# ssydasheng/GPflow-Slim

Measured on AMD Instinct MI355X. Metric: GPR log-marginal-likelihood evals/sec + predict_f latency, fp64, N=32768 D=8, higher is better.
Workload: dtype f64; 1 GPU; RBF(ARD) GPR log-marginal-likelihood, N=32768 D=8 R=1 fp64, X resident in HBM; n=32768, d=8, n_new=1024, parallelism=1 GPU (fused single-GPU path)

## Files before the change

gpflow-slim_amd/csrc/blas1.hip:

```cpp
#include "gps_common.hpp"

typedef double v2d __attribute__((ext_vector_type(2)));

__device__ __forceinline__ double wave_sum(double v) {
#pragma unroll
  for (int off = 32; off > 0; off >>= 1) v += __shfl_xor(v, off, 64);
  return v;
}

__global__ __launch_bounds__(256) void trsv_base_kernel(const double* __restrict__ LinvT,
                                                        double* __restrict__ y, i64 ldy) {
  __shared__ double ys[128];
  __shared__ double part[128];
  double* yr = y + (i64)blockIdx.x * ldy;
  const int tid = threadIdx.x, i = tid & 127, half = tid >> 7;
  if (tid < 128) ys[tid] = yr[tid];
  __syncthreads();
  const double* Lc = LinvT + (half * 64) * 128 + i;
  double s = 0.0;
#pragma unroll 16
  for (int c = 0; c < 64; ++c) s += Lc[c * 128] * ys[half * 64 + c];
  if (half) part[i] = s;
  __syncthreads();
  if (!half) yr[i] = s + part[i];
}

template <int RC>
__global__ __launch_bounds__(256) void gemv_sub_kernel(const double* __restrict__ L21, i64 ldl,
                                                       i64 n2, i64 n1,
                                                       const double* __restrict__ y1,
                                                       double* __restrict__ y2, i64 ldy, int r0,
                                                       int rcount) {
  const int lane = threadIdx.x & 63;
// ... 549 lines not shown
  const i64 row = (i64)blockIdx.x * 4 + (threadIdx.x >> 6);
  if (row >= rows) return;
  const double* a = A + row * lda; const double* b = B + row * ldb;
  double s = 0.0;
  for (i64 k = 2 * lane; k < cols; k += 128) {
    const v2d x = *reinterpret_cast<const v2d*>(a + k), y = *reinterpret_cast<const v2d*>(b + k);
    s = fma(x.x, y.x, fma(x.y, y.y, s));
  }
  s = wave_sum(s);
  if (lane == 0) out[row] = s;
}
__global__ __launch_bounds__(256) void rows_axpby_kernel(double* __restrict__ X, i64 ldx, const double* __restrict__ Y, i64 ldy,
                                                         i64 rows, i64 cols, const double* __restrict__ a, const double* __restrict__ b) {
  const i64 c = (i64)blockIdx.x * blockDim.x + threadIdx.x;
  if (c >= cols) return;
  for (i64 rr = blockIdx.y; rr < rows; rr += gridDim.y) X[rr * ldx + c] = a[rr] * X[rr * ldx + c] + b[rr] * Y[rr * ldy + c];
}
int gps_launch_rowdot2(gps_handle_t h, const double* A, i64 lda, const double* B, i64 ldb, i64 rows, i64 cols, double* out) {
  if (rows <= 0 || cols <= 0) return GPS_OK;
  LaunchScope ls(h, KC_REDUCE, 2.0 * rows * cols, 16.0 * rows * cols);
  hipLaunchKernelGGL(rowdot2_kernel, dim3((unsigned)((rows + 3) / 4)), dim3(256), 0, h->stream, A, lda, B, ldb, rows, cols, out);
  GPS_HIP(h, hipGetLastError());
  return GPS_OK;
}
int gps_launch_rows_axpby(gps_handle_t h, double* X, i64 ldx, const double* Y, i64 ldy, i64 rows, i64 cols, const double* a,
                          const double* b) {
  if (rows <= 0 || cols <= 0) return GPS_OK;
  LaunchScope ls(h, KC_OTHER, 3.0 * rows * cols, 24.0 * rows * cols);
  dim3 grid((unsigned)((cols + 255) / 256), (unsigned)(rows < 32768 ? rows : 32768));
  hipLaunchKernelGGL(rows_axpby_kernel, grid, dim3(256), 0, h->stream, X, ldx, Y, ldy, rows, cols, a, b);
  GPS_HIP(h, hipGetLastError());
  return GPS_OK;
}
int gps_launch_axpby_eye(gps_handle_t h, double* A, i64 ld, i64 n, i64 n_real, double alpha, double beta) {
  if (n <= 0) return GPS_OK;
  LaunchScope ls(h, KC_OTHER, (double)n * n, 16.0 * n * n);
  dim3 grid((unsigned)((n + 255) / 256), (unsigned)(n < 32768 ? n : 32768));
  hipLaunchKernelGGL(axpby_eye_kernel, grid, dim3(256), 0, h->stream, A, ld, n, n_real, alpha, beta);
  GPS_HIP(h, hipGetLastError());
  return GPS_OK;
}
int gps_launch_diag_recip_add(gps_handle_t h, double* A, i64 lda, const double* L, i64 ldl, i64 n, double coef) {
  if (n <= 0) return GPS_OK;
  hipLaunchKernelGGL(diag_recip_add_kernel, dim3((unsigned)((n + 255) / 256)), dim3(256), 0, h->stream, A, lda, L, ldl, n, coef);
  GPS_HIP(h, hipGetLastError());
  return GPS_OK;
}
int gps_tri_dot(gps_handle_t h, const double* A, i64 lda, const double* B, i64 ldb, i64 n, double* out2) {
  out2[0] = out2[1] = 0.0;
  if (n <= 0) return GPS_OK;
  double* part = h->dScal.d();
  {
    LaunchScope ls(h, KC_REDUCE, (double)n * n, 8.0 * n * n);
    hipLaunchKernelGGL(tri_dot_kernel, dim3(64), dim3(256), 0, h->stream, A, lda, B, ldb, n, part);
    GPS_HIP(h, hipGetLastError());
  }
  double hp[128];
  GPS_HIP(h, hipMemcpyAsync(hp, part, sizeof(hp), hipMemcpyDeviceToHost, h->stream));
  GPS_HIP(h, hipStreamSynchronize(h->stream));
  for (int b = 0; b < 64; ++b) { out2[0] += hp[2 * b]; out2[1] += hp[2 * b + 1]; }
  return GPS_OK;
}

int gps_launch_tri_map(gps_handle_t h, double* A, i64 ld, i64 n, int mode) {
  if (n <= 0) return GPS_OK;
  LaunchScope ls(h, KC_OTHER, (double)n * n, 16.0 * n * n);
// ... 169 lines not shown
```

gpflow-slim_amd/csrc/gemm_f64.hip:

```cpp
#include "gps_common.hpp"

typedef double v4d __attribute__((ext_vector_type(4)));
typedef double v2d __attribute__((ext_vector_type(2)));

#define BK_MIN 16
#ifndef STRIP
#define STRIP 8
#endif

struct GemmArgs {
  const double* A; const double* B; double* C;
  i64 lda, ldb, ldc;
  int Tm, Tn;
  int K;
  int ntiles;
  int triA;
  int batch, tpb;
  int pair;
  i64 a_rs, a_cs, b_rs, b_cs, c_rs, c_cs, a_cm, b_cm, c_cm;
  int cb_tiles;
  i64 cb_stride;
  int cb_cpack = 0;
  int nfull, nsplit;
  double* ws;
  unsigned* cnt;
  unsigned long long* sig_ptr; unsigned long long sig_val;
  long long* stamps;
};

__device__ __forceinline__ int xcd_remap(int b, int nb) {
#ifdef GPS_GEMM_NO_XCD_REMAP
  return b;
#endif
  const int q = nb >> 3, r = nb & 7;
  const int x = b & 7, idx = b >> 3;
  const int base = (x < r) ? x * (q + 1) : r * (q + 1) + (x - r) * q;
  return base + idx;
}

template <bool LOWER>
__device__ __forceinline__ void decode_tile(int id, int Tm, int Tn, int& tm, int& tn) {
  if (!LOWER) {
    const int full = Tn / STRIP;
    const int per = Tm * STRIP;
    int s = id / per;
    if (s >= full) {
      const int w = Tn - full * STRIP;
      const int rem = id - full * per;
      tm = rem / w; tn = full * STRIP + rem % w;
    } else {
      const int rem = id - s * per;
      tm = rem / STRIP; tn = s * STRIP + rem % STRIP;
    }
  } else {
    int s = 0, rem = id;
    for (;;) {
      const int c0 = s * STRIP;
      const int w = min(STRIP, Tn - c0);
      const int tri = w * (w + 1) / 2;
      const int cnt = tri + (Tm - c0 - w) * w;
      if (rem < cnt) {
        if (rem < tri) {
          int rr = 0;
          while (rem >= rr + 1) { rem -= rr + 1; ++rr; }
          tm = c0 + rr; tn = c0 + rem;
        } else {
          rem -= tri;
          tm = c0 + w + rem / w; tn = c0 + rem % w;
        }
        return;
      }
      rem -= cnt; ++s;
    }
  }
}

#define GEMM_KERNEL_NAME gemm_nt_f64_kernel
#define GEMM_PAIR_TPARAM
#include "gemm_f64_kernel.inc"
#undef GEMM_KERNEL_NAME
#undef GEMM_PAIR_TPARAM
#define GEMM_PAIRED
#define GEMM_KERNEL_NAME gemm_nt_f64_pair_kernel
#define GEMM_PAIR_TPARAM , int PAIR = 1
#include "gemm_f64_kernel.inc"
#undef GEMM_PAIRED
#undef GEMM_KERNEL_NAME
#undef GEMM_PAIR_TPARAM

template <int BM, int BN, int WGM, bool LOWER, int OP, int PIPE = 0, int BKT = 16>
static int launch_variant(gps_handle_t h, const GemmArgs& g) {
  const size_t lds = (size_t)(2 * (BM + BN) * (BKT + 2)) * sizeof(double);
  if (g.pair && BM == BN && PIPE == 2 && !LOWER && (OP == 1 || OP == 3)) {
    const int grid = g.ntiles;
    if (g.pair == 1) {
      int rc = gps_dyn_lds(h, reinterpret_cast<const void*>(&gemm_nt_f64_pair_kernel<BM, BN, WGM, false, OP, PIPE, BKT, 1>), (int)lds);
      if (rc) return rc;
      hipLaunchKernelGGL((gemm_nt_f64_pair_kernel<BM, BN, WGM, false, OP, PIPE, BKT, 1>), dim3(grid), dim3(256), lds, h->stream, g);
    } else {
      int rc = gps_dyn_lds(h, reinterpret_cast<const void*>(&gemm_nt_f64_pair_kernel<BM, BN, WGM, false, OP, PIPE, BKT, 2>), (int)lds);
      if (rc) return rc;
      hipLaunchKernelGGL((gemm_nt_f64_pair_kernel<BM, BN, WGM, false, OP, PIPE, BKT, 2>), dim3(grid), dim3(256), lds, h->stream, g);
    }
    GPS_HIP(h, hipGetLastError());
    return GPS_OK;
  }
  int rc = gps_dyn_lds(h, reinterpret_cast<const void*>(&gemm_nt_f64_kernel<BM, BN, WGM, LOWER, OP, PIPE, BKT>), (int)lds);
  if (rc) return rc;
  const int grid = g.nsplit > 1 ? g.nfull + (g.ntiles - g.nfull) * g.nsplit : g.ntiles;
  hipLaunchKernelGGL((gemm_nt_f64_kernel<BM, BN, WGM, LOWER, OP, PIPE, BKT>), dim3(grid), dim3(256), lds, h->stream, g);
  GPS_HIP(h, hipGetLastError());
// ... 98 lines not shown
  g.cb_tiles = 0; g.cb_stride = 0;
  const double t128 = (double)nbatch * (lower ? 0.5 * (double)(N / 128) * (double)(N / 128 + 1) + (double)((M - N) / 128) * (double)(N / 128)
                                             : ((double)M / 128.0) * (double)(N / 128));
  const double flops = triA == 3 ? (double)nbatch * 128.0 * 128.0 * ((double)M / 128.0) * (double)(N / 128) * (double)(N + 128)
                     : triA      ? (double)nbatch * 128.0 * 128.0 * (double)(N / 128) * (double)(M / 128) * (double)(M + 128)
                                 : 2.0 * t128 * 128.0 * 128.0 * (double)K;
  const double bytes = t128 * (((op == 0 || op == 2) ? 2.0 : 1.0) * 128.0 * 128.0 * 8.0) +
                       8.0 * (double)K * (double)(M + N);
  LaunchScope ls(h, KC_GEMM, flops, bytes);
  ls.tag[0] = M; ls.tag[1] = N; ls.tag[2] = K; ls.tag[3] = op + 10 * lower + 20 * triA + 100 * (rowpanel ? 1 : 0) + 1000 * (nbatch > 1 ? nbatch : 0);
  const double target = (double)h->gemm_min_tiles;
  const int force = h->gemm_force_tb;
  if (rowpanel) {
    int bm = 16;
    if (force) bm = (half_rows && force > 64) ? 64 : force;
    else if (M / 128 >= 256 && !half_rows) bm = 128;
    else if (M / 64 >= 256) bm = 64;
    else if (M / 32 >= 256) bm = 32;
    if (bm == 128) return launch_cfg<128, 128, 2>(h, op, 0, g, M, N);
    if (bm == 64) return launch_cfg<64, 128, 2>(h, op, 0, g, M, N);
    if (bm == 32) return launch_cfg<32, 128, 1>(h, op, 0, g, M, N);
    return launch_cfg<16, 128, 1>(h, op, 0, g, M, N);
  }
  int tb = 32;
  if (force) tb = force < 32 ? 32 : force;
  else if (t128 >= target && !half_rows) tb = 128;
  else if (4.0 * t128 >= target) tb = 64;
  if (half_rows && tb > 64) tb = 64;
  if (tb == 128) return launch_cfg<128, 128, 2>(h, op, lower, g, M, N);
  if (tb == 64) return launch_cfg<64, 64, 2>(h, op, lower, g, M, N);
  return launch_cfg<32, 32, 2>(h, op, lower, g, M, N);
}

int gps_launch_gemm_nt_cyclic(gps_handle_t h, i64 M, i64 nblocks, i64 nb, i64 stride, i64 K, const double* A, i64 lda,
                              double* C, i64 ldc, int c_packed) {
  if (M <= 0 || nblocks <= 0) return GPS_OK;
  if (M % 128 || nb % 128 || stride % 128 || K % BK_MIN || stride < nb || (nblocks - 1) * stride + nb > M)
    return gps_fail(h, GPS_ERR_ARG, "gemm_nt_cyclic: sizes must be multiples of 128 and the blocks must lie inside the panel");
  GemmArgs g;
  g.A = A; g.B = A; g.C = C; g.lda = lda; g.ldb = lda; g.ldc = ldc; g.K = (int)K; g.triA = 0;
  g.batch = 1; g.tpb = 0; g.pair = 0; g.a_rs = g.a_cs = g.b_rs = g.b_cs = g.c_rs = g.c_cs = g.a_cm = g.b_cm = g.c_cm = 0;
  g.sig_ptr = nullptr; g.sig_val = 0;
  g.stamps = h->gemm_stamps;
  double t128 = 0.0;
  for (i64 b = 0; b < nblocks; ++b) { const i64 rows = M - b * stride; if (rows > 0) t128 += (double)(rows / 128) * (double)(nb / 128); }
  const double flops = 2.0 * t128 * 128.0 * 128.0 * (double)K;
  LaunchScope ls(h, KC_GEMM, flops, t128 * 2.0 * 128.0 * 128.0 * 8.0 + 8.0 * (double)K * (double)(M + nblocks * nb));
  const double target = (double)h->gemm_min_tiles;
  g.cb_stride = stride;
  g.cb_cpack = c_packed ? 1 : 0;
  if (t128 >= target) { g.cb_tiles = (int)(nb / 128); return launch_cfg<128, 128, 2>(h, 0, 0, g, M, nblocks * nb); }
  if (4.0 * t128 >= target) { g.cb_tiles = (int)(nb / 64); return launch_cfg<64, 64, 2>(h, 0, 0, g, M, nblocks * nb); }
  g.cb_tiles = (int)(nb / 32);
  return launch_cfg<32, 32, 2>(h, 0, 0, g, M, nblocks * nb);
}
```

gpflow-slim_amd/csrc/gemm_f64_kernel.inc:

```
template <int BM, int BN, int WGM, bool LOWER, int OP, int PIPE = 0, int BKT = 16 GEMM_PAIR_TPARAM>
__global__ __launch_bounds__(256, 2) void GEMM_KERNEL_NAME(GemmArgs g) {
  constexpr int BK = BKT, LS = BKT + 2;
  constexpr int TPR = BKT / 2, RPP = 256 / TPR;
  constexpr int WGN = 4 / WGM;
  constexpr int WTM = BM / WGM, WTN = BN / WGN;
  constexpr int MI = WTM / 16, NI = WTN / 16;
  constexpr int LPA = (BM + RPP - 1) / RPP, LPB = (BN + RPP - 1) / RPP;
  static_assert(MI >= 1 && NI >= 1, "wave tile must hold at least one MFMA tile");
  constexpr int KS = (MI * NI >= 4) ? 1 : (MI * NI == 2 ? 2 : 4);
  extern __shared__ __attribute__((aligned(16))) char smem_raw[];
  double* As = reinterpret_cast<double*>(smem_raw);
  double* Bs = As + 2 * BM * LS;

  int tile_id, slice = -1, tail = 0;
  if ((int)blockIdx.x < g.nfull || g.nsplit <= 1) {
    tile_id = xcd_remap((int)blockIdx.x, g.nsplit > 1 ? g.nfull : g.ntiles);
  } else {
    const int q = (int)blockIdx.x - g.nfull;
    tail = q / g.nsplit;
    slice = q - tail * g.nsplit;
    tile_id = g.nfull + tail;
  }
  int tm, tn;
  i64 bcol;
  const double* gA = g.A; const double* gB = g.B; double* gC = g.C;
  if (g.batch > 1) {
    const int p = tile_id / g.tpb;
    tile_id -= p * g.tpb;
    gA += (i64)p * g.a_rs * g.lda + (g.a_cm ? ((i64)p * g.a_cs) % g.a_cm : (i64)p * g.a_cs);
    gB += (i64)p * g.b_rs * g.ldb + (g.b_cm ? ((i64)p * g.b_cs) % g.b_cm : (i64)p * g.b_cs);
    gC += (i64)p * g.c_rs * g.ldc + (g.c_cm ? ((i64)p * g.c_cs) % g.c_cm : (i64)p * g.c_cs);
  }
  if (g.cb_tiles > 0) {
    const int q = (int)(g.cb_stride / BM);
// ... 228 lines not shown
          for (int rg = 0; rg < 4; ++rg) acc[0][i][j][rg] += v[i][j][rg];
    }
    if (tid == 0) g.cnt[tail] = 0;
  }
  const i64 row0 = (i64)tm * BM + wr * WTM + (lane >> 4);
  const i64 col0 = (g.cb_cpack ? (i64)tn * BN : bcol) + wc * WTN + (lane & 15);
  constexpr int IB = (MI >= 2) ? 2 : 1;
#pragma unroll
  for (int i0 = 0; i0 < MI; i0 += IB) {
    double cv[IB][NI][4];
    if (OP == 0 || OP == 2) {
#pragma unroll
      for (int ii = 0; ii < IB; ++ii)
#pragma unroll
        for (int j = 0; j < NI; ++j)
#pragma unroll
          for (int rg = 0; rg < 4; ++rg)
            cv[ii][j][rg] = gC[(row0 + (i0 + ii) * 16 + 4 * rg) * g.ldc + col0 + j * 16];
    }
#pragma unroll
    for (int ii = 0; ii < IB; ++ii)
#pragma unroll
      for (int j = 0; j < NI; ++j)
#pragma unroll
        for (int rg = 0; rg < 4; ++rg) {
          double* cp = gC + (row0 + (i0 + ii) * 16 + 4 * rg) * g.ldc + col0 + j * 16;
          const double av = acc[0][i0 + ii][j][rg];
          if (OP == 0) *cp = cv[ii][j][rg] - av;
          else if (OP == 2) *cp = cv[ii][j][rg] + av;
          else if (OP == 3) *cp = -av;
          else *cp = av;
        }
  }
#ifdef GEMM_PAIRED
  }
#endif
  if (g.stamps && threadIdx.x == 0) g.stamps[6 * (long long)blockIdx.x + 1] = (long long)wall_clock64();
}
```

gpflow-slim_amd/csrc/gps_common.hpp:

```cpp
#pragma once
#include <hip/hip_runtime.h>
#include <cstdint>
#include <cstdio>
#include <cstring>
#include <cstdlib>
#include <string>
#include <vector>
#include "../../include/gpflowslim_hip.h"
#include "blocked.hpp"

#define GPS_TILE 128
#define GPS_WB 2048
#define GPS_WIDE_MAX_ROWS 8192

typedef int64_t i64;

static inline i64 gps_pad(i64 n) { return ((n + GPS_TILE - 1) / GPS_TILE) * GPS_TILE; }

struct DevBuf;
typedef std::vector<DevBuf*> DevBufList;
struct DevBuf {
  enum Class { WORK, PERSISTENT };
  void*  p = nullptr;
  size_t cap = 0;
// ... 172 lines not shown
  DevBuf dA{bufs};
  DevBuf dY{bufs};
  DevBuf dKinv{bufs};
  DevBuf dS1{bufs}, dS2{bufs}, dS3{bufs}, dS4{bufs};
  DevBuf dG1{bufs}, dG2{bufs}, dG3{bufs}, dG4{bufs};
  DevBuf dLikIn{bufs}, dLikOut{bufs}, dLikPart{bufs}, dLikH{bufs};
  DevBuf dTmp{bufs};
  DevBuf dTmp2{bufs};
  DevBuf dTmp3{bufs};
  static constexpr long long resid_ring_max = 1 << 16;
  int trsm_panel = 1;
  int trsm_tall_ratio = 16;
  int trsm_panel_rows = 0;
  DevBuf dSmallOut{bufs};
  DevBuf dFeatG{bufs};
  DevBuf dGradSums{bufs};
  void* hRes = nullptr;
  DevBuf dBlkCond{bufs};
  DevBuf dSmallSync{bufs, DevBuf::PERSISTENT};
  static constexpr i64 small_n_max = 2048;
  struct SmallPath {
    int on = 1;
    int fault_inject = 0;
    long long fallbacks = 0;
    int consec = 0;
    int cooldown = 0;
    bool defer = false;
    bool pending = false;
    bool valid = false;
    double slog = 0.0, ssq = 0.0;
    bool linvT_stale = false;
  } small;
  DevBuf dGemmWs{bufs}, dGemmCnt{bufs};
  struct RffFactor { bool have = false; unsigned long long gen = 0; i64 F = 0, r = 0; int kind = -1, d = 0; bool refine = false; } rff;
  DevBuf dGemvWs{bufs}, dGemvCnt{bufs};
  struct KgprSolve { bool have = false; unsigned long long gen = 0; i64 m = 0, n = 0; } kgpr;
  int kron_cg_check_every = 8;
};

static inline int gps_fail(gps_handle_t h, int code, const std::string& msg) {
  if (h) h->err = msg;
  return code;
}

static inline int gps_dyn_lds(gps_handle_t h, const void* fn, int bytes);

#define GPS_HIP(h, call)                                                         \
  do {                                                                           \
    hipError_t e__ = (call);                                                     \
    if (e__ != hipSuccess) {                                                     \
      return gps_fail(h, GPS_ERR_HIP, std::string(#call) + ": " + hipGetErrorString(e__)); \
    }                                                                            \
  } while (0)

static inline void drop_resident_factors(gps_handle_t h) {
  h->have_factor = false; h->factor_gen++; h->dist.have_part_factor = false; h->dist.grad_ready = false;
}

#define DIST_TAIL 4
struct DistPanel {
  i64 np, nb, ld;
  i64 rows;
  i64 blk0, nbb;
  i64 below;
  double* panel;
  i64 inv_doubles() const { return nbb * GPS_TILE * GPS_TILE; }
// ... 52 lines not shown
    hipEvent_t e; (void)hipEventCreate(&e); return e;
  }
};

static inline void gps_profile_collect(gps_handle_t h) {
  static const char* dump_path = getenv("GPS_PROF_DUMP");
  FILE* df = (dump_path && !h->pending.empty()) ? fopen(dump_path, "a") : nullptr;
  for (auto& p : h->pending) {
    float ms = 0.f;
    if (hipEventElapsedTime(&ms, p.a, p.b) == hipSuccess) h->stat[p.klass].ms += ms;
    if (df) fprintf(df, "%s %lld %lld %lld %lld %.3f\n", kc_names[p.klass], (long long)p.t[0], (long long)p.t[1], (long long)p.t[2], (long long)p.t[3], 1e3 * ms);
    h->evt_pool.push_back(p.a); h->evt_pool.push_back(p.b);
  }
  if (df) fclose(df);
  h->pending.clear();
}

static inline int gps_dyn_lds(gps_handle_t h, const void* fn, int bytes) {
  for (const void* f : h->dyn_lds_done) if (f == fn) return GPS_OK;
  GPS_HIP(h, hipFuncSetAttribute(fn, hipFuncAttributeMaxDynamicSharedMemorySize, bytes));
  h->dyn_lds_done.push_back(fn);
  return GPS_OK;
}

int gps_launch_gemm_nt(gps_handle_t h, int op, int lower, i64 M, i64 N, i64 K,
                       const double* A, i64 lda, const double* B, i64 ldb,
                       double* C, i64 ldc);
struct GemmBatch;
int gps_launch_gemm_nt_ex(gps_handle_t h, int op, int lower, int tri, i64 M, i64 N, i64 K,
                          const double* A, i64 lda, const double* B, i64 ldb,
                          double* C, i64 ldc, const GemmBatch* bt);
int gps_launch_gemm_nt_cyclic(gps_handle_t h, i64 M, i64 nblocks, i64 nb, i64 stride, i64 K, const double* A, i64 lda,
                              double* C, i64 ldc, int c_packed = 0);
int gps_launch_potrf_base(gps_handle_t h, double* A, i64 lda, double* Linv_blk,
                          double* LinvT_blk, int* d_info, i64 row0, int factor,
                          long long* d_stamps = nullptr);
int gps_launch_trsm_leaf_refine(gps_handle_t h, double* B, i64 ldb, i64 m, const double* W, const double* D, i64 ldd,
                                int upper);
int gps_launch_trsv_leaf_refine(gps_handle_t h, const double* Wt, const double* D, i64 ldd, double* y, i64 ldy, i64 r,
                                int upper);
static inline bool gps_gpr_needs_refine(const gps_handle_s* h, double noise_var, double kdiag, i64 n) {
  if (h->leaf_refine >= 0) return h->leaf_refine > 0;
  return !((double)n * kdiag + noise_var <= h->leaf_refine_cond * noise_var);
}

struct SmallKgen { int on = 0; int op = 0; const double* X = nullptr; int d_all = 0; int nd = 0; int dims[16]; double inv_ls[16]; double variance = 0.0, noise = 0.0; };
int gps_launch_small_factor(gps_handle_t h, double* dK, i64 np, double* linv, double* linvT, const double* d_resid, i64 n, i64 r,
                            int* d_info, double* d_res4, double* d_alpha, i64 ld_alpha, i64 alpha_rows, const SmallKgen* kgen = nullptr);
int gps_small_factor_reset(gps_handle_t h);
int gps_launch_trsm_panel(gps_handle_t h, double* B, i64 ldb, i64 m, const double* L, i64 ldl, const double* W, int backward);
int gps_launch_small_inverse(gps_handle_t h, const double* dK, i64 np, const double* linv, const double* d_alpha, i64 r,
                             double* dY, double* dKinv, double* dA, double* d_res1, double* dAT = nullptr, i64 n = 0);
int gps_launch_trsv_wave(gps_handle_t h, const double* L, i64 ldl, i64 n, const double* W, double* y, i64 ldy, i64 r,
                         int trans, int refine = 0);
int gps_launch_trsv_base(gps_handle_t h, const double* Linv_blk, double* y, i64 ldy, i64 r);
int gps_launch_la_wait(gps_handle_t h, hipStream_t st, unsigned long long* sig, unsigned long long sval,
                       const unsigned long long* flag, unsigned long long val, unsigned long long* timeouts);
int gps_launch_gemv_sub(gps_handle_t h, const double* L21, i64 ldl, i64 n2, i64 n1,
                        const double* y1, double* y2, i64 ldy, i64 r);
int gps_launch_gemv_t_sub(gps_handle_t h, const double* L21, i64 ldl, i64 n2, i64 n1,
                          const double* y2, double* y1, i64 ldy, i64 r);
int gps_launch_lml_reduce(gps_handle_t h, const double* L, i64 ldl, i64 n,
                          const double* alpha, i64 ldy, i64 r, double* out2);
int gps_launch_colsumsq(gps_handle_t h, const double* A, i64 ld, i64 rows, i64 cols, double* sumsq);
int gps_launch_rowdot(gps_handle_t h, const double* At, i64 ldat, i64 n_new, i64 npad,
                      const double* alpha, i64 ldy, i64 r, double* mean, double* sumsq);
// ... 118 lines not shown
```

gpflow-slim_amd/csrc/gps_handle.hip:

```cpp
#include "gps_ops.hpp"

extern "C" int gps_create(int device_id, gps_handle_t* out) {
  if (!out) return GPS_ERR_ARG;
  *out = nullptr;
  int count = 0;
  if (hipGetDeviceCount(&count) != hipSuccess || count <= 0) return GPS_ERR_HIP;
  if (device_id < 0 || device_id >= count) return GPS_ERR_ARG;
  gps_handle_t h = new gps_handle_s();
  h->device = device_id;
  if (hipSetDevice(device_id) != hipSuccess || hipGetDeviceProperties(&h->prop, device_id) != hipSuccess) {
    delete h;
    return GPS_ERR_HIP;
  }
  if (hipStreamCreateWithFlags(&h->stream, hipStreamNonBlocking) != hipSuccess) { delete h; return GPS_ERR_HIP; }
  for (int i = 0; i < 8; ++i) {
    if (hipEventCreate(&h->ev[i]) != hipSuccess) { delete h; return GPS_ERR_HIP; }
  }
  if (const char* v = getenv("GPS_GEMM_PAIR")) h->gemm_pair = atoi(v);
  if (const char* la = getenv("GPS_LOOKAHEAD")) h->potrf_lookahead = atoi(la);
  if (h->dInfo.ensure(64) != hipSuccess || h->dScal.ensure(4096) != hipSuccess) { delete h; return GPS_ERR_HIP; }
  *out = h;
  return GPS_OK;
}

// ... 77 lines not shown
    {"trsv_wave_fallbacks", (long long)h->wave_fallbacks},
  };
  for (const auto& c : counters) {
    if (strcmp(klass, c.key) != 0) continue;
    if (launches) *launches = (int64_t)c.value;
    if (ms) *ms = 0.0;
    if (flops) *flops = 0.0;
    if (bytes) *bytes = 0.0;
    return GPS_OK;
  }
  GPS_HIP(h, hipStreamSynchronize(h->stream));
  gps_profile_collect(h);
  for (int i = 0; i < KC_COUNT; ++i) {
    if (strcmp(klass, kc_names[i]) == 0) {
      if (launches) *launches = h->stat[i].launches;
      if (ms) *ms = h->stat[i].ms;
      if (flops) *flops = h->stat[i].flops;
      if (bytes) *bytes = h->stat[i].bytes;
      return GPS_OK;
    }
  }
  return gps_fail(h, GPS_ERR_ARG, "unknown kernel class");
}
extern "C" int gps_last_stage_ms(gps_handle_t h, double* out5) {
  if (!h || !out5) return GPS_ERR_ARG;
  for (int i = 0; i < 5; ++i) out5[i] = h->stage_ms[i];
  return GPS_OK;
}

extern "C" int gps_set_option(gps_handle_t h, const char* key, double value) {
  if (!h || !key) return GPS_ERR_ARG;
  if (strcmp(key, "gemm_force_tile") == 0) { h->gemm_force_tb = (int)value; return GPS_OK; }
  if (strcmp(key, "gemm_tail_split") == 0) { h->gemm_tail_split = (int)value; return GPS_OK; }
  if (strcmp(key, "kmat_fast") == 0) { h->kmat_fast = (int)value; return GPS_OK; }
  if (strcmp(key, "kmat_mfma") == 0) { h->kmat_mfma = (int)value; return GPS_OK; }
  if (strcmp(key, "trsv_wave") == 0) { h->trsv_wave = (int)value; return GPS_OK; }
  if (strcmp(key, "gpr_aug_rows") == 0) { h->gpr_aug_rows = (int)value; return GPS_OK; }
  if (strcmp(key, "leaf_refine") == 0) { h->leaf_refine = (int)value; return GPS_OK; }
  if (strcmp(key, "potrf_rl_max") == 0) { h->potrf_rl_max = (int)value; return GPS_OK; }
  if (strcmp(key, "potrf_lookahead") == 0) { h->potrf_lookahead = (int)value; return GPS_OK; }
  if (strcmp(key, "la_fault_inject") == 0) { h->la_fault_inject = (int)value; return GPS_OK; }
  if (strcmp(key, "wave_fault_inject") == 0) { h->wave_fault_inject = (int)value; return GPS_OK; }
  if (strcmp(key, "small_fault_inject") == 0) { h->small.fault_inject = (int)value; return GPS_OK; }
  if (strcmp(key, "svgp_kl_weight") == 0) { h->svgp_kl_weight = value; return GPS_OK; }
  if (strcmp(key, "dist_partitioned") == 0) { h->dist.partitioned = (int)value; return GPS_OK; }
  if (strcmp(key, "leaf_plain_kappa") == 0) { h->leaf_plain_kappa = value; h->plain_linv = nullptr; return GPS_OK; }
  if (strcmp(key, "follower_max_wgs") == 0) { h->follower_max_wgs = (int)value; return GPS_OK; }
  if (strcmp(key, "potrf_rl_group") == 0) { h->potrf_rl_group = (int)value < 1 ? 1 : (int)value; return GPS_OK; }
  if (strcmp(key, "small_n") == 0) { h->small.on = (int)value; return GPS_OK; }
  if (strcmp(key, "trsm_panel") == 0) { h->trsm_panel = (int)value; return GPS_OK; }
  if (strcmp(key, "trsm_tall_ratio") == 0) { h->trsm_tall_ratio = (int)value; return GPS_OK; }
  if (strcmp(key, "trsm_panel_rows") == 0) {
    if (value != 0 && value != 32 && value != 64 && value != 65) return gps_fail(h, GPS_ERR_ARG, "trsm_panel_rows: 0, 32, 64 or 65");
    h->trsm_panel_rows = (int)value; return GPS_OK;
  }
  if (strcmp(key, "predict_inverse_blocks") == 0) { h->predict_inv_blocks = (int)value; return GPS_OK; }
  if (strcmp(key, "trsv_wave_refine") == 0) { h->trsv_wave_refine = (int)value; return GPS_OK; }
  if (strcmp(key, "kron_cg_check_every") == 0) { h->kron_cg_check_every = (int)value < 1 ? 1 : (int)value; return GPS_OK; }
  return gps_fail(h, GPS_ERR_ARG, "unknown option");
}

extern "C" int gps_diag_mfma_f64(gps_handle_t h, int waves_per_simd, double* tflops, int* layout_ok) {
  if (!h) return GPS_ERR_ARG;
  GPS_HIP(h, hipSetDevice(h->device));
  return gps_run_mfma_diag(h, waves_per_simd, tflops, layout_ok);
}

extern "C" int gps_diag_gemm_nt(gps_handle_t h, int op, int lower, int64_t m, int64_t n, int64_t k,
                                const double* A, const double* B, double* C) {
  if (!h || !A || !B || !C) return GPS_ERR_ARG;
  GPS_HIP(h, hipSetDevice(h->device));
  const size_t ab = (size_t)m * k * 8, bb = (size_t)n * k * 8, cb = (size_t)m * n * 8;
  GPS_HIP(h, h->dTmp.ensure(ab)); GPS_HIP(h, h->dTmp2.ensure(bb)); GPS_HIP(h, h->dTmp3.ensure(cb));
  GPS_HIP(h, hipMemcpyAsync(h->dTmp.p, A, ab, hipMemcpyHostToDevice, h->stream));
  GPS_HIP(h, hipMemcpyAsync(h->dTmp2.p, B, bb, hipMemcpyHostToDevice, h->stream));
  GPS_HIP(h, hipMemcpyAsync(h->dTmp3.p, C, cb, hipMemcpyHostToDevice, h->stream));
  int rc = lower >= 3 ? gps_launch_gemm_nt_ex(h, op, 0, lower - 1, m, n, k, h->dTmp.d(), k, h->dTmp2.d(), k, h->dTmp3.d(), n, nullptr)
                      : gps_launch_gemm_nt(h, op, lower, m, n, k, h->dTmp.d(), k, h->dTmp2.d(), k, h->dTmp3.d(), n);
  if (rc) return rc;
  GPS_HIP(h, hipMemcpyAsync(C, h->dTmp3.p, cb, hipMemcpyDeviceToHost, h->stream));
  GPS_HIP(h, hipStreamSynchronize(h->stream));
  return GPS_OK;
}

extern "C" int gps_diag_gemm_nt_batched(gps_handle_t h, int op, int tri, int64_t batch, int64_t m, int64_t n, int64_t k,
                                        const double* A, const double* B, double* C) {
  if (!h || !A || !B || !C || batch < 1) return GPS_ERR_ARG;
  GPS_HIP(h, hipSetDevice(h->device));
  const size_t ab = (size_t)batch * m * k * 8, bb = (size_t)batch * n * k * 8, cb = (size_t)batch * m * n * 8;
  GPS_HIP(h, h->dTmp.ensure(ab)); GPS_HIP(h, h->dTmp2.ensure(bb)); GPS_HIP(h, h->dTmp3.ensure(cb));
  GPS_HIP(h, hipMemcpyAsync(h->dTmp.p, A, ab, hipMemcpyHostToDevice, h->stream));
  GPS_HIP(h, hipMemcpyAsync(h->dTmp2.p, B, bb, hipMemcpyHostToDevice, h->stream));
  GPS_HIP(h, hipMemcpyAsync(h->dTmp3.p, C, cb, hipMemcpyHostToDevice, h->stream));
  GemmBatch bt; bt.batch = batch; bt.a_rs = m; bt.b_rs = n; bt.c_rs = m;
  int rc = gps_launch_gemm_nt_ex(h, op, 0, tri, m, n, k, h->dTmp.d(), k, h->dTmp2.d(), k, h->dTmp3.d(), n, &bt);
  if (rc) return rc;
  GPS_HIP(h, hipMemcpyAsync(C, h->dTmp3.p, cb, hipMemcpyDeviceToHost, h->stream));
  GPS_HIP(h, hipStreamSynchronize(h->stream));
  return GPS_OK;
}

extern "C" int gps_diag_gemm_timeline(gps_handle_t h, int op, int lower, int64_t m, int64_t n, int64_t k, int reps,
                                      long long* stamps_out, int64_t cap_blocks, int64_t* nblocks, double* ms_per_launch) {
  if (!h || !stamps_out || cap_blocks <= 0 || reps <= 0) return GPS_ERR_ARG;
  GPS_HIP(h, hipSetDevice(h->device));
  return gps_run_gemm_timeline(h, op, lower, m, n, k, reps, stamps_out, cap_blocks, nblocks, ms_per_launch);
}

extern "C" int gps_diag_potrf_base_stamps(gps_handle_t h, int factor, double* us_out7) {
  if (!h || !us_out7) return GPS_ERR_ARG;
  GPS_HIP(h, hipSetDevice(h->device));
// ... 231 lines not shown
```

gpflow-slim_amd/csrc/gps_ops.hpp:

```cpp
#pragma once
#include "gps_common.hpp"
#include "blocked.hpp"
#include "dist_schedule.hpp"
#include <climits>
#include <cmath>
#include <algorithm>

struct HipOps {
  gps_handle_t h;
  double* linv;
  double* linvT;
  int* d_info;
  int factor = 1;
  bool store_T = true;

  int potrf_base(double* A, i64 lda, i64 blk, i64 row0) {
    if (h->plain_linv == linv) h->plain_linv = nullptr;
    return gps_launch_potrf_base(h, A, lda, linv + blk * GPS_TILE * GPS_TILE,
                                 (linvT && store_T) ? linvT + blk * GPS_TILE * GPS_TILE : nullptr, d_info, row0,
                                 factor);
  }
  int trsm_base(i64 blk, int transposed, double* B, i64 ldb, i64 m, const double* D, i64 ldd) {
    const double* W = (transposed ? linvT : linv) + blk * GPS_TILE * GPS_TILE;
    if (h->refine_now && !plain_ok(blk, 1)) { h->leaves_refined++; return gps_launch_trsm_leaf_refine(h, B, ldb, m, W, D, ldd, transposed); }
    if (h->refine_now) h->leaves_plain++;
    return gps_launch_gemm_nt(h,  1, 0, m, GPS_TILE, GPS_TILE, B, ldb, W, GPS_TILE, B, ldb);
  }
  bool plain_ok(i64 blk, i64 cnt) const {
    if (h->plain_linv != linv || blk < 0 || (size_t)(blk + cnt) > h->plain_flags.size()) return false;
    for (i64 b = blk; b < blk + cnt; ++b) if (!h->plain_flags[(size_t)b]) return false;
    return true;
  }
  bool trsm_left_looking(i64 m, i64 n) const { return h->trsm_tall_ratio > 0 && m >= (i64)h->trsm_tall_ratio * n; }
  bool leaf512(i64 m, int transposed, i64 blk) const {
    return h->trsm_panel > 0 && (!h->refine_now || plain_ok(blk, 4)) && m >= 64 && m % 64 == 0 && (transposed ? linvT != nullptr : true);
  }
  int trsm_leaf512(i64 blk, int transposed, double* B, i64 ldb, i64 m, const double* D, i64 ldd) {
    if (h->refine_now) h->leaves_plain += 4;
    const double* W = (transposed ? linvT : linv) + blk * GPS_TILE * GPS_TILE;
    return gps_launch_trsm_panel(h, B, ldb, m, D, ldd, W, transposed);
  }
  int gemm(int op, int lower, i64 M, i64 N, i64 K, const double* A, i64 lda, const double* B,
           i64 ldb, double* C, i64 ldc) {
    if (h->follower_max_wgs > 0 && op == 0 && !lower && h->def_stream && h->stream == h->def_stream && M >= 128 && N > 128) {
      const i64 rows = (M + 127) / 128;
      const i64 w = std::max<i64>(1, h->follower_max_wgs / rows) * 128;
      if (w < N) {
        for (i64 u = 0; u < N; u += w) {
          const int rc = gps_launch_gemm_nt(h, op, lower, M, std::min(w, N - u), K, A, lda, B + u * ldb, ldb, C + u, ldc);
          if (rc) return rc;
        }
        return GPS_OK;
      }
    }
    return gps_launch_gemm_nt(h, op, lower, M, N, K, A, lda, B, ldb, C, ldc);
  }
  int gemm_ex(int op, int tri, i64 M, i64 N, i64 K, const double* A, i64 lda, const double* B, i64 ldb, double* C, i64 ldc, const GemmBatch* bt) {
    return gps_launch_gemm_nt_ex(h, op, 0, tri, M, N, K, A, lda, B, ldb, C, ldc, bt);
  }
  int blocks_to_diag(const double* src, double* dst, i64 nblk, i64 wb) { return gps_launch_blocks_to_diag(h, src, dst, nblk, wb); }
  int trsv_base(i64 blk, double* y, i64 ldy, i64 r, const double* D, i64 ldd) {
    if (!linvT) return gps_fail(h, GPS_ERR_STATE, "trsv needs the transposed block inverses");
    if (h->refine_now) return gps_launch_trsv_leaf_refine(h, linvT + blk * GPS_TILE * GPS_TILE, D, ldd, y, ldy, r, 0);
    return gps_launch_trsv_base(h, linvT + blk * GPS_TILE * GPS_TILE, y, ldy, r);
  }
  int gemv_sub(const double* L21, i64 ldl, i64 n2, i64 n1, const double* y1, double* y2, i64 ldy,
               i64 r) {
    return gps_launch_gemv_sub(h, L21, ldl, n2, n1, y1, y2, ldy, r);
  }
  int trsv_t_base(i64 blk, double* y, i64 ldy, i64 r, const double* D, i64 ldd) {
    if (h->refine_now) return gps_launch_trsv_leaf_refine(h, linv + blk * GPS_TILE * GPS_TILE, D, ldd, y, ldy, r, 1);
    return gps_launch_trsv_base(h, linv + blk * GPS_TILE * GPS_TILE, y, ldy, r);
  }
  int gemv_t_sub(const double* L21, i64 ldl, i64 n2, i64 n1, const double* y2, double* y1, i64 ldy, i64 r) {
    return gps_launch_gemv_t_sub(h, L21, ldl, n2, n1, y2, y1, ldy, r);
  }
// ... 287 lines not shown
```

Before: 5.525 evals/s.

## Apply one-level Strassen to large fp64 NT GEMM updates with dual-output epilogue

Large non-triangular GEMM updates on the main stream, and the off-diagonal half of large lower-triangular updates, are routed through a one-level Strassen scheme. It uses seven half-size products instead of eight. A new dual-target GEMM kernel variant writes each product to two C quadrants in its epilogue, and a vectorized block-add kernel forms the operand sums. The goal is to cut fp64 matrix-core work in the dominant Cholesky trailing updates. The cost is extra memory traffic for the operand sums and the second-target read-modify-write, plus a small loss of numerical accuracy from Strassen in fp64.

```diff
diff --git a/gpflow-slim_amd/csrc/blas1.hip b/gpflow-slim_amd/csrc/blas1.hip
--- a/gpflow-slim_amd/csrc/blas1.hip
+++ b/gpflow-slim_amd/csrc/blas1.hip
@@ -1,4 +1,5 @@
 #include "gps_common.hpp"
+#include <algorithm>
 
 typedef double v2d __attribute__((ext_vector_type(2)));
 
@@ -614,6 +615,40 @@
   GPS_HIP(h, hipGetLastError());
   return GPS_OK;
 }
+typedef double sum_v2d __attribute__((ext_vector_type(2)));
+__global__ __launch_bounds__(256) void block_sum_kernel(double* __restrict__ D, i64 ldd, const double* __restrict__ X, i64 ldx,
+                                                        const double* __restrict__ Y, i64 ldy, i64 rows, i64 cols2, double sign) {
+  for (i64 c = (i64)blockIdx.x * blockDim.x + threadIdx.x; c < cols2; c += (i64)gridDim.x * blockDim.x) {
+    i64 rr = blockIdx.y;
+    for (; rr + 3 * (i64)gridDim.y < rows; rr += 4 * (i64)gridDim.y) {
+      sum_v2d x[4], y[4];
+#pragma unroll
+      for (int u = 0; u < 4; ++u) {
+        x[u] = *reinterpret_cast<const sum_v2d*>(X + (rr + u * (i64)gridDim.y) * ldx + 2 * c);
+        y[u] = *reinterpret_cast<const sum_v2d*>(Y + (rr + u * (i64)gridDim.y) * ldy + 2 * c);
+      }
+#pragma unroll
+      for (int u = 0; u < 4; ++u) *reinterpret_cast<sum_v2d*>(D + (rr + u * (i64)gridDim.y) * ldd + 2 * c) = x[u] + sign * y[u];
+    }
+    for (; rr < rows; rr += gridDim.y)
+      *reinterpret_cast<sum_v2d*>(D + rr * ldd + 2 * c) =
+          *reinterpret_cast<const sum_v2d*>(X + rr * ldx + 2 * c) + sign * *reinterpret_cast<const sum_v2d*>(Y + rr * ldy + 2 * c);
+  }
+}
+int gps_launch_block_sum(gps_handle_t h, double* D, i64 ldd, const double* X, i64 ldx, const double* Y, i64 ldy, i64 rows, i64 cols,
+                         int sign) {
+  if (rows <= 0 || cols <= 0) return GPS_OK;
+  if ((cols & 1) || (ldd & 1) || (ldx & 1) || (ldy & 1) || (((uintptr_t)D | (uintptr_t)X | (uintptr_t)Y) & 15))
+    return gps_fail(h, GPS_ERR_ARG, "block_sum: blocks must be 16-byte aligned with even widths and leading dimensions");
+  LaunchScope ls(h, KC_GEMM, (double)rows * (double)cols, 24.0 * (double)rows * (double)cols);
+  ls.tag[0] = rows; ls.tag[1] = cols; ls.tag[3] = -1;
+  const i64 cols2 = cols / 2;
+  const unsigned gx = (unsigned)std::min<i64>((cols2 + 255) / 256, 64);
+  const unsigned gy = (unsigned)std::min<i64>(rows, std::max<i64>(1, 4096 / gx));
+  hipLaunchKernelGGL(block_sum_kernel, dim3(gx, gy), dim3(256), 0, h->stream, D, ldd, X, ldx, Y, ldy, rows, cols2, sign < 0 ? -1.0 : 1.0);
+  GPS_HIP(h, hipGetLastError());
+  return GPS_OK;
+}
 int gps_launch_axpby_eye(gps_handle_t h, double* A, i64 ld, i64 n, i64 n_real, double alpha, double beta) {
   if (n <= 0) return GPS_OK;
   LaunchScope ls(h, KC_OTHER, (double)n * n, 16.0 * n * n);
diff --git a/gpflow-slim_amd/csrc/gemm_f64.hip b/gpflow-slim_amd/csrc/gemm_f64.hip
--- a/gpflow-slim_amd/csrc/gemm_f64.hip
+++ b/gpflow-slim_amd/csrc/gemm_f64.hip
@@ -26,6 +26,7 @@
   unsigned* cnt;
   unsigned long long* sig_ptr; unsigned long long sig_val;
   long long* stamps;
+  double* C2 = nullptr; i64 ldc2 = 0; int op2 = 0;
 };
 
 __device__ __forceinline__ int xcd_remap(int b, int nb) {
@@ -76,7 +77,7 @@
 }
 
 #define GEMM_KERNEL_NAME gemm_nt_f64_kernel
-#define GEMM_PAIR_TPARAM
+#define GEMM_PAIR_TPARAM , bool DUAL = false
 #include "gemm_f64_kernel.inc"
 #undef GEMM_KERNEL_NAME
 #undef GEMM_PAIR_TPARAM
@@ -241,6 +242,37 @@
   return launch_cfg<32, 32, 2>(h, op, lower, g, M, N);
 }
 
+int gps_launch_gemm_nt_dual(gps_handle_t h, i64 M, i64 N, i64 K, const double* A, i64 lda, const double* B, i64 ldb,
+                            double* C, i64 ldc, double* C2, i64 ldc2, int op2) {
+  if (M <= 0 || N <= 0 || K <= 0) return GPS_OK;
+  if (M % 128 || N % 128 || K % BK_MIN || !C || !C2 || (op2 != 0 && op2 != 2))
+    return gps_fail(h, GPS_ERR_ARG, "gemm_nt_dual: M,N must be multiples of 128 and K of 16, two targets, op2 0 or 2");
+  if ((lda & 1) || (ldb & 1) || ((uintptr_t)A & 15) || ((uintptr_t)B & 15))
+    return gps_fail(h, GPS_ERR_ARG, "gemm_nt_dual: operands must be 16-byte aligned with even leading dimension");
+  if (C == A || C2 == A || C == C2) return gps_fail(h, GPS_ERR_ARG, "gemm_nt_dual: no in-place form");
+  if ((M / 128) * (N / 128) > 0x7fffffff) return gps_fail(h, GPS_ERR_ARG, "gemm_nt: too many tiles");
+  GemmArgs g;
+  g.A = A; g.B = B; g.C = C; g.lda = lda; g.ldb = ldb; g.ldc = ldc; g.K = (int)K; g.triA = 0;
+  g.batch = 1; g.pair = 0;
+  g.a_rs = g.a_cs = g.b_rs = g.b_cs = g.c_rs = g.c_cs = g.a_cm = g.b_cm = g.c_cm = 0;
+  g.cb_tiles = 0; g.cb_stride = 0;
+  g.Tm = (int)(M / 128); g.Tn = (int)(N / 128);
+  g.ntiles = g.Tm * g.Tn; g.tpb = g.ntiles;
+  g.nfull = g.ntiles; g.nsplit = 1; g.ws = nullptr; g.cnt = nullptr;
+  g.stamps = nullptr;
+  g.sig_ptr = h->next_sig_ptr; g.sig_val = h->next_sig_val; h->next_sig_ptr = nullptr;
+  g.C2 = C2; g.ldc2 = ldc2; g.op2 = op2;
+  const double t128 = (double)g.ntiles;
+  LaunchScope ls(h, KC_GEMM, 2.0 * t128 * 128.0 * 128.0 * (double)K, t128 * 4.0 * 128.0 * 128.0 * 8.0 + 8.0 * (double)K * (double)(M + N));
+  ls.tag[0] = M; ls.tag[1] = N; ls.tag[2] = K; ls.tag[3] = 50 + op2;
+  const size_t lds = (size_t)(2 * (128 + 128) * (16 + 2)) * sizeof(double);
+  int rc = gps_dyn_lds(h, reinterpret_cast<const void*>(&gemm_nt_f64_kernel<128, 128, 2, false, 0, 2, 16, true>), (int)lds);
+  if (rc) return rc;
+  hipLaunchKernelGGL((gemm_nt_f64_kernel<128, 128, 2, false, 0, 2, 16, true>), dim3(g.ntiles), dim3(256), lds, h->stream, g);
+  GPS_HIP(h, hipGetLastError());
+  return GPS_OK;
+}
+
 int gps_launch_gemm_nt_cyclic(gps_handle_t h, i64 M, i64 nblocks, i64 nb, i64 stride, i64 K, const double* A, i64 lda,
                               double* C, i64 ldc, int c_packed) {
   if (M <= 0 || nblocks <= 0) return GPS_OK;
diff --git a/gpflow-slim_amd/csrc/gemm_f64_kernel.inc b/gpflow-slim_amd/csrc/gemm_f64_kernel.inc
--- a/gpflow-slim_amd/csrc/gemm_f64_kernel.inc
+++ b/gpflow-slim_amd/csrc/gemm_f64_kernel.inc
@@ -1,5 +1,8 @@
 template <int BM, int BN, int WGM, bool LOWER, int OP, int PIPE = 0, int BKT = 16 GEMM_PAIR_TPARAM>
 __global__ __launch_bounds__(256, 2) void GEMM_KERNEL_NAME(GemmArgs g) {
+#ifdef GEMM_PAIRED
+  constexpr bool DUAL = false;
+#endif
   constexpr int BK = BKT, LS = BKT + 2;
   constexpr int TPR = BKT / 2, RPP = 256 / TPR;
   constexpr int WGN = 4 / WGM;
@@ -294,6 +297,30 @@
           else *cp = av;
         }
   }
+  if (DUAL) {
+    double* gC2 = g.C2;
+    const bool sub2 = g.op2 == 0;
+#pragma unroll
+    for (int i0 = 0; i0 < MI; i0 += IB) {
+      double cv[IB][NI][4];
+#pragma unroll
+      for (int ii = 0; ii < IB; ++ii)
+#pragma unroll
+        for (int j = 0; j < NI; ++j)
+#pragma unroll
+          for (int rg = 0; rg < 4; ++rg)
+            cv[ii][j][rg] = gC2[(row0 + (i0 + ii) * 16 + 4 * rg) * g.ldc2 + col0 + j * 16];
+#pragma unroll
+      for (int ii = 0; ii < IB; ++ii)
+#pragma unroll
+        for (int j = 0; j < NI; ++j)
+#pragma unroll
+          for (int rg = 0; rg < 4; ++rg) {
+            const double av = acc[0][i0 + ii][j][rg];
+            gC2[(row0 + (i0 + ii) * 16 + 4 * rg) * g.ldc2 + col0 + j * 16] = sub2 ? cv[ii][j][rg] - av : cv[ii][j][rg] + av;
+          }
+    }
+  }
 #ifdef GEMM_PAIRED
   }
 #endif
diff --git a/gpflow-slim_amd/csrc/gps_common.hpp b/gpflow-slim_amd/csrc/gps_common.hpp
--- a/gpflow-slim_amd/csrc/gps_common.hpp
+++ b/gpflow-slim_amd/csrc/gps_common.hpp
@@ -228,6 +228,8 @@
     bool linvT_stale = false;
   } small;
   DevBuf dGemmWs{bufs}, dGemmCnt{bufs};
+  int gemm_strassen_min = 4096;
+  DevBuf dStrS{bufs}, dStrT{bufs};
   struct RffFactor { bool have = false; unsigned long long gen = 0; i64 F = 0, r = 0; int kind = -1, d = 0; bool refine = false; } rff;
   DevBuf dGemvWs{bufs}, dGemvCnt{bufs};
   struct KgprSolve { bool have = false; unsigned long long gen = 0; i64 m = 0, n = 0; } kgpr;
@@ -346,6 +348,10 @@
                           double* C, i64 ldc, const GemmBatch* bt);
 int gps_launch_gemm_nt_cyclic(gps_handle_t h, i64 M, i64 nblocks, i64 nb, i64 stride, i64 K, const double* A, i64 lda,
                               double* C, i64 ldc, int c_packed = 0);
+int gps_launch_gemm_nt_dual(gps_handle_t h, i64 M, i64 N, i64 K, const double* A, i64 lda, const double* B, i64 ldb,
+                            double* C, i64 ldc, double* C2, i64 ldc2, int op2);
+int gps_launch_block_sum(gps_handle_t h, double* D, i64 ldd, const double* X, i64 ldx, const double* Y, i64 ldy, i64 rows, i64 cols,
+                         int sign);
 int gps_launch_potrf_base(gps_handle_t h, double* A, i64 lda, double* Linv_blk,
                           double* LinvT_blk, int* d_info, i64 row0, int factor,
                           long long* d_stamps = nullptr);
diff --git a/gpflow-slim_amd/csrc/gps_handle.hip b/gpflow-slim_amd/csrc/gps_handle.hip
--- a/gpflow-slim_amd/csrc/gps_handle.hip
+++ b/gpflow-slim_amd/csrc/gps_handle.hip
@@ -133,6 +133,10 @@
   if (!h || !key) return GPS_ERR_ARG;
   if (strcmp(key, "gemm_force_tile") == 0) { h->gemm_force_tb = (int)value; return GPS_OK; }
   if (strcmp(key, "gemm_tail_split") == 0) { h->gemm_tail_split = (int)value; return GPS_OK; }
+  if (strcmp(key, "gemm_strassen_min") == 0) {
+    if (value < 0 || value != (double)((i64)value) || (i64)value % 128) return gps_fail(h, GPS_ERR_ARG, "gemm_strassen_min: 0 or a multiple of 128");
+    h->gemm_strassen_min = (int)value; return GPS_OK;
+  }
   if (strcmp(key, "kmat_fast") == 0) { h->kmat_fast = (int)value; return GPS_OK; }
   if (strcmp(key, "kmat_mfma") == 0) { h->kmat_mfma = (int)value; return GPS_OK; }
   if (strcmp(key, "trsv_wave") == 0) { h->trsv_wave = (int)value; return GPS_OK; }
@@ -176,8 +180,11 @@
   GPS_HIP(h, hipMemcpyAsync(h->dTmp.p, A, ab, hipMemcpyHostToDevice, h->stream));
   GPS_HIP(h, hipMemcpyAsync(h->dTmp2.p, B, bb, hipMemcpyHostToDevice, h->stream));
   GPS_HIP(h, hipMemcpyAsync(h->dTmp3.p, C, cb, hipMemcpyHostToDevice, h->stream));
+  h->refine_now = false;
+  HipOps ops{h, nullptr, nullptr, nullptr};
   int rc = lower >= 3 ? gps_launch_gemm_nt_ex(h, op, 0, lower - 1, m, n, k, h->dTmp.d(), k, h->dTmp2.d(), k, h->dTmp3.d(), n, nullptr)
-                      : gps_launch_gemm_nt(h, op, lower, m, n, k, h->dTmp.d(), k, h->dTmp2.d(), k, h->dTmp3.d(), n);
+         : lower == 2 ? gps_launch_gemm_nt(h, op, lower, m, n, k, h->dTmp.d(), k, h->dTmp2.d(), k, h->dTmp3.d(), n)
+                      : ops.gemm(op, lower, m, n, k, h->dTmp.d(), k, h->dTmp2.d(), k, h->dTmp3.d(), n);
   if (rc) return rc;
   GPS_HIP(h, hipMemcpyAsync(C, h->dTmp3.p, cb, hipMemcpyDeviceToHost, h->stream));
   GPS_HIP(h, hipStreamSynchronize(h->stream));
diff --git a/gpflow-slim_amd/csrc/gps_ops.hpp b/gpflow-slim_amd/csrc/gps_ops.hpp
--- a/gpflow-slim_amd/csrc/gps_ops.hpp
+++ b/gpflow-slim_amd/csrc/gps_ops.hpp
@@ -1,6 +1,7 @@
 #pragma once
 #include "gps_common.hpp"
 #include "blocked.hpp"
+#include "strassen.hpp"
 #include "dist_schedule.hpp"
 #include <climits>
 #include <cmath>
@@ -40,8 +41,37 @@
     const double* W = (transposed ? linvT : linv) + blk * GPS_TILE * GPS_TILE;
     return gps_launch_trsm_panel(h, B, ldb, m, D, ldd, W, transposed);
   }
+  bool on_main_stream() const {
+    if (saved_stream || saved_stream_d) return false;
+    if (h->side_stream && h->stream == h->side_stream) return false;
+    if (h->def_stream && h->stream == h->def_stream) return false;
+    if (h->dist.bulk_set && h->stream == h->dist.bulk_stream) return false;
+    return true;
+  }
   int gemm(int op, int lower, i64 M, i64 N, i64 K, const double* A, i64 lda, const double* B,
            i64 ldb, double* C, i64 ldc) {
+    const i64 smin = h->gemm_strassen_min;
+    if (smin > 0 && op == 0 && !h->refine_now && C != A && on_main_stream()) {
+      if (lower == 0 && strassen_shape_ok(M, N, K, smin)) {
+        GPS_HIP(h, h->dStrS.ensure((size_t)(M / 2) * (size_t)(K / 2) * 8));
+        GPS_HIP(h, h->dStrT.ensure((size_t)(N / 2) * (size_t)(K / 2) * 8));
+        const int rc = strassen_nt(*this, M, N, K, A, lda, B, ldb, C, ldc, h->dStrS.d(), h->dStrT.d());
+        return rc < 0 ? gps_fail(h, GPS_ERR_ARG, "strassen_nt: bad shape") : rc;
+      }
+      int rc = 0;
+      if (lower == 1 && strassen_lower_split(*this, M, N, K, A, lda, B, ldb, C, ldc, smin, &rc)) return rc;
+    }
+    return gemm_plain(op, lower, M, N, K, A, lda, B, ldb, C, ldc);
+  }
+  int add(double* D, i64 ldd, const double* X, i64 ldx, const double* Y, i64 ldy, i64 rows, i64 cols, int sign) {
+    return gps_launch_block_sum(h, D, ldd, X, ldx, Y, ldy, rows, cols, sign);
+  }
+  int gemm2(i64 M, i64 N, i64 K, const double* A, i64 lda, const double* B, i64 ldb, double* C, i64 ldc, double* C2, i64 ldc2, int op2) {
+    if (!C2) return gps_launch_gemm_nt(h, 0, 0, M, N, K, A, lda, B, ldb, C, ldc);
+    return gps_launch_gemm_nt_dual(h, M, N, K, A, lda, B, ldb, C, ldc, C2, ldc2, op2);
+  }
+  int gemm_plain(int op, int lower, i64 M, i64 N, i64 K, const double* A, i64 lda, const double* B,
+                 i64 ldb, double* C, i64 ldc) {
     if (h->follower_max_wgs > 0 && op == 0 && !lower && h->def_stream && h->stream == h->def_stream && M >= 128 && N > 128) {
       const i64 rows = (M + 127) / 128;
       const i64 w = std::max<i64>(1, h->follower_max_wgs / rows) * 128;
diff --git a/gpflow-slim_amd/csrc/strassen.hpp b/gpflow-slim_amd/csrc/strassen.hpp
--- /dev/null
+++ b/gpflow-slim_amd/csrc/strassen.hpp
@@ -0,0 +1,54 @@
+#pragma once
+#include <cstdint>
+
+template <class Ops>
+int strassen_nt(Ops& ops, int64_t M, int64_t N, int64_t K, const double* A, int64_t lda, const double* B, int64_t ldb, double* C,
+                int64_t ldc, double* S, double* T) {
+  typedef int64_t i64;
+  if (M <= 0 || N <= 0 || K <= 0) return 0;
+  if (M % 256 || N % 256 || K % 256) return -1;
+  const i64 m = M / 2, n = N / 2, k = K / 2;
+  const double* A11 = A;            const double* A12 = A + k;
+  const double* A21 = A + m * lda;  const double* A22 = A21 + k;
+  const double* B11 = B;            const double* B12 = B + k;
+  const double* B21 = B + n * ldb;  const double* B22 = B21 + k;
+  double* C11 = C;            double* C12 = C + n;
+  double* C21 = C + m * ldc;  double* C22 = C21 + n;
+  int rc;
+  if ((rc = ops.add(S, k, A11, lda, A22, lda, m, k, +1))) return rc;
+  if ((rc = ops.add(T, k, B11, ldb, B22, ldb, n, k, +1))) return rc;
+  if ((rc = ops.gemm2(m, n, k, S, k, T, k, C11, ldc, C22, ldc, 0))) return rc;
+  if ((rc = ops.add(S, k, A21, lda, A22, lda, m, k, +1))) return rc;
+  if ((rc = ops.gemm2(m, n, k, S, k, B11, ldb, C21, ldc, C22, ldc, 2))) return rc;
+  if ((rc = ops.add(T, k, B21, ldb, B22, ldb, n, k, -1))) return rc;
+  if ((rc = ops.gemm2(m, n, k, A11, lda, T, k, C12, ldc, C22, ldc, 0))) return rc;
+  if ((rc = ops.add(T, k, B12, ldb, B11, ldb, n, k, -1))) return rc;
+  if ((rc = ops.gemm2(m, n, k, A22, lda, T, k, C11, ldc, C21, ldc, 0))) return rc;
+  if ((rc = ops.add(S, k, A11, lda, A12, lda, m, k, +1))) return rc;
+  if ((rc = ops.gemm2(m, n, k, S, k, B22, ldb, C12, ldc, C11, ldc, 2))) return rc;
+  if ((rc = ops.add(S, k, A21, lda, A11, lda, m, k, -1))) return rc;
+  if ((rc = ops.add(T, k, B11, ldb, B21, ldb, n, k, +1))) return rc;
+  if ((rc = ops.gemm2(m, n, k, S, k, T, k, C22, ldc, nullptr, 0, 0))) return rc;
+  if ((rc = ops.add(S, k, A12, lda, A22, lda, m, k, -1))) return rc;
+  if ((rc = ops.add(T, k, B12, ldb, B22, ldb, n, k, +1))) return rc;
+  return ops.gemm2(m, n, k, S, k, T, k, C11, ldc, nullptr, 0, 0);
+}
+
+static inline bool strassen_shape_ok(int64_t M, int64_t N, int64_t K, int64_t min_quadrant) {
+  if (min_quadrant <= 0 || M % 256 || N % 256 || K % 256) return false;
+  return M / 2 >= min_quadrant && N / 2 >= min_quadrant && K / 2 >= min_quadrant;
+}
+
+template <class Ops>
+bool strassen_lower_split(Ops& ops, int64_t M, int64_t N, int64_t K, const double* A, int64_t lda, const double* B, int64_t ldb,
+                          double* C, int64_t ldc, int64_t min_quadrant, int* rc_out) {
+  typedef int64_t i64;
+  const i64 n = N / 2;
+  if (min_quadrant <= 0 || M < N || N % 256 || n / 2 < min_quadrant || !strassen_shape_ok(n, n, K, min_quadrant)) return false;
+  int rc = ops.gemm_plain(0, 1, n, n, K, A, lda, B, ldb, C, ldc);
+  if (!rc) rc = ops.gemm(0, 0, n, n, K, A + n * lda, lda, B, ldb, C + n * ldc, ldc);
+  if (!rc && M > N) rc = ops.gemm_plain(0, 0, M - N, n, K, A + N * lda, lda, B, ldb, C + N * ldc, ldc);
+  if (!rc) rc = ops.gemm_plain(0, 1, M - n, n, K, A + n * lda, lda, B + n * ldb, ldb, C + n * ldc + n, ldc);
+  *rc_out = rc;
+  return true;
+}
```

Measured after the change: 5.642 evals/s, median of 6. 1.02x the previous value.
